# visionworkbench/visionworkbench

Hardware: AMD Instinct MI355X
Metric: disparity Mpix/s, 4096x4096 pair, 7x7 SAD, +-64-px search (higher is better)
Workload: dtype u8

## Files before the change

visionworkbench_amd/csrc/bm_sad_u8.hip:

```cpp
#include <climits>
#include <cstdlib>
#include <type_traits>

#include "vwgpu_internal.h"
#include "u8_tile.h"

#ifdef VWGPU_TILE_STAMPS
__device__ unsigned long long* g_sad_stamps = nullptr;
extern "C" int vwgpu_debug_set_sad_stamps(void* d_buf) {
  unsigned long long* p = static_cast<unsigned long long*>(d_buf);
  return hipMemcpyToSymbol(HIP_SYMBOL(g_sad_stamps), &p, sizeof p) == hipSuccess ? 0 : -3;
}
#define VWGPU_STAMP(k) do { if (g_sad_stamps && tid == 0) g_sad_stamps[(size_t)wg * 16 + (k)] = wall_clock64(); } while (0)
#else
#define VWGPU_STAMP(k) do { } while (0)
#endif

namespace {

using namespace vwgpu_u8;
typedef uint32_t u32;
typedef uint64_t u64;
typedef unsigned short u16x2 __attribute__((ext_vector_type(2)));

__device__ __forceinline__ u32 pk_sub_u16(u32 a, u32 b) {
  return __builtin_bit_cast(u32, (u16x2)(__builtin_bit_cast(u16x2, a) - __builtin_bit_cast(u16x2, b)));
}
__device__ __forceinline__ u32 pk_max_u16(u32 a, u32 b) {
  return __builtin_bit_cast(u32, __builtin_elementwise_max(__builtin_bit_cast(u16x2, a), __builtin_bit_cast(u16x2, b)));
}
__device__ __forceinline__ u32 pk_min_u16(u32 a, u32 b) {
  return __builtin_bit_cast(u32, __builtin_elementwise_min(__builtin_bit_cast(u16x2, a), __builtin_bit_cast(u16x2, b)));
}
__device__ __forceinline__ void umin3_acc(u32& k, u32 a, u32 b) {
  asm volatile("v_min3_u32 %0, %0, %1, %2" : "+v"(k) : "v"(a), "v"(b));
}

template <int W>
__device__ __forceinline__ void key_sub(u32& key, u32 a, u32 b) {
  if (W == 0)
    asm volatile("v_sub_u16_sdwa %0, %1, %2 dst_sel:WORD_1 dst_unused:UNUSED_PRESERVE src0_sel:WORD_0 src1_sel:WORD_0"
                 : "+v"(key) : "v"(a), "v"(b));
  else
    asm volatile("v_sub_u16_sdwa %0, %1, %2 dst_sel:WORD_1 dst_unused:UNUSED_PRESERVE src0_sel:WORD_1 src1_sel:WORD_1"
                 : "+v"(key) : "v"(a), "v"(b));
}

template <int KX, int KY, int TY, int WV = 0>
struct Cfg {
  static constexpr int NW = (KX + 3) / 4;
  static constexpr int EW = NW <= 2 ? 2 : 4;
  static constexpr int WAVES = WV ? WV : (NW <= 2 ? 4 : 2);
  static constexpr int THREADS = WAVES * 64;
  static constexpr int TWB = WAVES * 256;
  static constexpr int NR = TY + KY - 1;
  static constexpr int LBW = TWB / 4 + NW + 1;
  static constexpr u32 LAST_MASK = (KX % 4 == 0) ? 0xffffffffu : ((1u << (8 * (KX % 4))) - 1u);
};

__device__ __forceinline__ void divmod_small(int idx, int d, float inv, int& quo, int& rem) {
  int qq = (int)(((float)idx + 0.5f) * inv);
  int rr = idx - qq * d;
  if (rr < 0) { --qq; rr += d; }
  if (rr >= d) { ++qq; rr -= d; }
  quo = qq; rem = rr;
}

__device__ __forceinline__ bool sad_second_on_cu(unsigned block, int first_round) {
  return (int)(block >> 3) >= (first_round >> 4);
}

__host__ __device__ constexpr size_t ent_words(int nr, int ne, int ew, int gr, int ty, int pt) {
  const size_t ent = (size_t)nr * ne * ew;
  const size_t merge = gr > 1 ? (size_t)(gr - 1) * (ty / gr) * 4 * pt + (size_t)gr * pt : 0;
  const size_t ob = (size_t)gr * (pt / 64) * 768;
  return ent > merge ? (ent > ob ? ent : ob) : (merge > ob ? merge : ob);
}

template <int KX, int KY, int TY, int GR, int WV = 0, bool EM = true>
__global__ void __launch_bounds__((GR * (Cfg<KX, KY, TY, WV>::THREADS)), (GR > 1 ? 1 : (TY <= 8 && KX <= 8 ? 3 : 2)))
bm_sad_u8_kernel(const float* __restrict__ L, ptrdiff_t ls, int lw, int lh,
                 const float* __restrict__ R, ptrdiff_t rs, int rcw, int rch,
                 int sx, int sy, int ne, int32_t* __restrict__ out, ptrdiff_t os, int ow, int oh,
                 int* __restrict__ flag_set, int* __restrict__ flag_clear,
                 int gxt, int ntiles, int last_round, int first_round, int stagger_ticks) {
  typedef Cfg<KX, KY, TY, WV> C;
  constexpr bool SPLIT = GR > 1;
  constexpr int NW = C::NW, EW = C::EW, NR = C::NR;
  constexpr int NRP = EM ? (NR | 1) : NR;
  extern __shared__ __attribute__((aligned(16))) u32 lds[];
  u32* ent = lds;
  const int bpitch = ne + NW + 1;
  u32* base = lds + ent_words(NRP, ne, EW, GR, TY, C::THREADS);
  u32* item_ctr = base + (size_t)NR * bpitch;

  constexpr int PT = C::THREADS;
  constexpr int NT = GR * PT;
  const int tid = threadIdx.x;
  const int grp = SPLIT ? __builtin_amdgcn_readfirstlane(tid / PT) : 0;
  const int ltid = SPLIT ? tid % PT : tid;
  const int pair_id = __builtin_amdgcn_readfirstlane(ltid >> 6);
  const int per_xcd = gridDim.x >> 3;
  const int wg = (int)(blockIdx.x & 7) * per_xcd + (int)(blockIdx.x >> 3);
  if (wg >= ntiles) return;
  const int x0 = (wg % gxt) * C::TWB;
  const int y0 = (wg / gxt) * TY;
  const int q = x0 + 4 * ltid;
  u32 bad_acc = 0;
  if (wg == 0 && tid == 0) *flag_clear = 0;
#ifdef VWGPU_TILE_STAMPS
  if (g_sad_stamps && tid == 0) {
    unsigned hw, xcc;
    asm volatile("s_getreg_b32 %0, hwreg(HW_REG_HW_ID)" : "=s"(hw));
    asm volatile("s_getreg_b32 %0, hwreg(HW_REG_XCC_ID)" : "=s"(xcc));
    unsigned long long* rec = g_sad_stamps + (size_t)wg * 16;
    rec[0] = wall_clock64(); rec[1] = clock64(); rec[2] = ((unsigned long long)xcc << 32) | hw;
  }
#endif

  if (!SPLIT && (int)blockIdx.x < first_round && sad_second_on_cu(blockIdx.x, first_round)) {
    if (tid < 64) {
      const u64 t_start = wall_clock64();
      for (int it = 0; it < 512 && wall_clock64() - t_start < (u64)stagger_ticks; ++it) __builtin_amdgcn_s_sleep(8);
    }
    __syncthreads();
  }
  stage_u8_rows<NR>(L, ls, lw, lh, x0, y0, C::LBW, C::LBW, ent, tid, NT, bad_acc);
  stage_u8_rows<NR>(R, rs, rcw, rch, x0, y0, bpitch, bpitch, base, tid, NT, bad_acc);
  __syncthreads();
  u64 win[NR][NW];
#pragma unroll
  for (int r = 0; r < NR; ++r) {
    u32 a[NW + 1];
#pragma unroll
    for (int n = 0; n <= NW; ++n) a[n] = ent[r * C::LBW + ltid + n];
#pragma unroll
    for (int n = 0; n < NW; ++n) win[r][n] = (u64)a[n] | ((u64)a[n + 1] << 32);
  }

  VWGPU_STAMP(3);
  u32 K[TY][4];
  u32 MN[TY][2], MX[TY][2];
#pragma unroll
  for (int y = 0; y < TY; ++y) K[y][0] = K[y][1] = K[y][2] = K[y][3] = 0xffffffffu;
  u32 eq_rows = (1u << TY) - 1u;
  int eq_checks = 0;
  constexpr int NPROBE = 4;
  const u32 zero = 0;

  const bool late = !SPLIT && (int)blockIdx.x >= last_round;
  if (!SPLIT) { if (late) __builtin_amdgcn_s_setprio(2); else __builtin_amdgcn_s_setprio(3); }
  typedef std::true_type T;
  typedef std::false_type F;

  auto sweep = [&](auto max_tag) __attribute__((always_inline)) {
    constexpr bool MAXSWEEP = decltype(max_tag)::value;
    for (int dy = 0; dy < sy; ++dy) {
      __syncthreads();
      if (dy > 0 || (MAXSWEEP && sy > 1)) stage_u8_rows<NR>(R, rs, rcw, rch, x0, y0 + dy, bpitch, bpitch, base, tid, NT, bad_acc);
      for (int t = 0; t < 4; ++t) {
        const int a_last = (sx + 2 - t) >> 2;
        __syncthreads();
        if (!MAXSWEEP && !SPLIT && dy == 0 && late) {
          if (t == 2) __builtin_amdgcn_s_setprio(1);
          else if (t == 3) __builtin_amdgcn_s_setprio(0);
        }
        {
          auto build = [&](int r, int m) __attribute__((always_inline)) {
            const u32* bp = base + (size_t)r * bpitch + m;
            u32 b[NW + 1];
#pragma unroll
            for (int n = 0; n <= NW; ++n) b[n] = bp[n];
            u32 w[EW];
#pragma unroll
            for (int n = 0; n < EW; ++n) w[n] = 0;
#pragma unroll
            for (int n = 0; n < NW; ++n) w[n] = __builtin_amdgcn_alignbyte(b[n + 1], b[n], t);
            w[NW - 1] &= C::LAST_MASK;
            u32* e = ent + (EM ? (size_t)m * NRP + r : (size_t)r * ne + m) * EW;
            if (EW == 2) *reinterpret_cast<uint2*>(e) = make_uint2(w[0], w[1]);
            else *reinterpret_cast<uint4*>(e) = make_uint4(w[0], w[1], w[2 % EW], w[3 % EW]);
          };
#pragma unroll 4
          for (int r = grp; r < NR; r += NT / PT) build(r, ltid);
          const int rem = ne - PT, total = NR * rem;
          const float inv = 1.0f / (float)rem;
          for (int idx = tid; idx < total; idx += NT) {
            int r, m;
            divmod_small(idx, rem, inv, r, m);
            build(r, PT + m);
          }
          if (SPLIT && tid < PT / 64) item_ctr[tid] = 0u;
        }
        __syncthreads();

        auto step = [&](int a, auto masked_tag, auto pair_tag, auto probe_tag) __attribute__((always_inline)) {
          constexpr bool MASKED = decltype(masked_tag)::value;
          constexpr bool PAIR = decltype(pair_tag)::value;
          constexpr bool PROBE = decltype(probe_tag)::value;
          const int jbase = 4 * a + t;
          const int ibase = dy * sx + jbase;
          u32 kinA[4], kinB[4];
          u32 orA[2] = {0u, 0u};
#pragma unroll
          for (int i = 0; i < 4; ++i) {
            kinA[i] = (u32)(ibase - i) & 0xffffu;
            kinB[i] = (u32)(ibase + 4 - i) & 0xffffu;
            if (MASKED) {
              const int d = jbase - i;
              if (d < 0 || d >= sx) orA[i >> 1] |= (i & 1) ? 0xffff0000u : 0x0000ffffu;
            }
          }
          const u32* ep = ent + (size_t)(ltid + a) * (EM ? NRP * EW : EW);
          u64 accA = 0, accB = 0;
          u64 PA[NR], PB[NR];
          constexpr int PF = 4;
          u32 wa[NR][EW], wb[NR][EW];
          auto fetch = [&](int r) __attribute__((always_inline)) {
            const u32* e = ep + (EM ? (size_t)r * EW : (size_t)r * ne * EW);
            constexpr int NX = EM ? NRP * EW : EW;
            if (EW == 2) {
              const uint2 v = *reinterpret_cast<const uint2*>(e);
              wa[r][0] = v.x; wa[r][1] = v.y;
              if (PAIR) { const uint2 u = *reinterpret_cast<const uint2*>(e + NX); wb[r][0] = u.x; wb[r][1] = u.y; }
            } else {
              const uint4 v = *reinterpret_cast<const uint4*>(e);
              wa[r][0] = v.x; wa[r][1] = v.y; wa[r][2 % EW] = v.z; wa[r][3 % EW] = v.w;
              if (PAIR) { const uint4 u = *reinterpret_cast<const uint4*>(e + NX); wb[r][0] = u.x; wb[r][1] = u.y; wb[r][2 % EW] = u.z; wb[r][3 % EW] = u.w; }
            }
          };
#pragma unroll
          for (int r = 0; r < PF && r < NR; ++r) fetch(r);
#pragma unroll
          for (int r = 0; r < NR; ++r) {
            if (r + PF < NR) fetch(r + PF);
#pragma unroll
            for (int n = 0; n < NW; ++n) {
              accA = __builtin_amdgcn_qsad_pk_u16_u8(win[r][n], wa[r][n], accA);
              if (PAIR) accB = __builtin_amdgcn_qsad_pk_u16_u8(win[r][n], wb[r][n], accB);
            }
            PA[r] = accA;
            if (PAIR) PB[r] = accB;
            if (r >= KY - 1) {
              const int y = r - (KY - 1);
              const int ro = (r >= KY) ? r - KY : 0;
              const u32 nA0 = (u32)PA[r], nA1 = (u32)(PA[r] >> 32);
              const u32 oA0 = (r >= KY) ? (u32)PA[ro] : zero;
              const u32 oA1 = (r >= KY) ? (u32)(PA[ro] >> 32) : zero;
              if (MAXSWEEP) {
                const u32 sA0 = pk_sub_u16(nA0, oA0), sA1 = pk_sub_u16(nA1, oA1);
                MN[y][0] = pk_min_u16(MN[y][0], MASKED ? (sA0 | orA[0]) : sA0);
                MN[y][1] = pk_min_u16(MN[y][1], MASKED ? (sA1 | orA[1]) : sA1);
                MX[y][0] = pk_max_u16(MX[y][0], MASKED ? (sA0 & ~orA[0]) : sA0);
                MX[y][1] = pk_max_u16(MX[y][1], MASKED ? (sA1 & ~orA[1]) : sA1);
                if (PAIR) {
                  const u32 nB0 = (u32)PB[r], nB1 = (u32)(PB[r] >> 32);
                  const u32 oB0 = (r >= KY) ? (u32)PB[ro] : zero;
                  const u32 oB1 = (r >= KY) ? (u32)(PB[ro] >> 32) : zero;
                  const u32 sB0 = pk_sub_u16(nB0, oB0), sB1 = pk_sub_u16(nB1, oB1);
                  MN[y][0] = pk_min_u16(MN[y][0], sB0);
                  MN[y][1] = pk_min_u16(MN[y][1], sB1);
                  MX[y][0] = pk_max_u16(MX[y][0], sB0);
                  MX[y][1] = pk_max_u16(MX[y][1], sB1);
                }
              } else {
                key_sub<0>(kinA[0], nA0, oA0); key_sub<1>(kinA[1], nA0, oA0);
                key_sub<0>(kinA[2], nA1, oA1); key_sub<1>(kinA[3], nA1, oA1);
                if (PAIR) {
                  const u32 nB0 = (u32)PB[r], nB1 = (u32)(PB[r] >> 32);
                  const u32 oB0 = (r >= KY) ? (u32)PB[ro] : zero;
                  const u32 oB1 = (r >= KY) ? (u32)(PB[ro] >> 32) : zero;
                  key_sub<0>(kinB[0], nB0, oB0); key_sub<1>(kinB[1], nB0, oB0);
                  key_sub<0>(kinB[2], nB1, oB1); key_sub<1>(kinB[3], nB1, oB1);
                  if (PROBE) {
                    u32 x[4];
#pragma unroll
                    for (int i = 0; i < 4; ++i) {
                      asm volatile("v_xor_b32 %0, %1, %2" : "=v"(x[i]) : "v"(kinA[i]), "v"(kinB[i]));
                      x[i] = (q + i < ow) ? x[i] : 0xffffffffu;
                    }
                    const u32 m01 = x[0] < x[1] ? x[0] : x[1], m23 = x[2] < x[3] ? x[2] : x[3];
                    if ((m01 < m23 ? m01 : m23) >> 16) eq_rows &= ~(1u << y);
                  }
                  umin3_acc(K[y][0], kinA[0], kinB[0]);
                  umin3_acc(K[y][1], kinA[1], kinB[1]);
                  umin3_acc(K[y][2], kinA[2], kinB[2]);
                  umin3_acc(K[y][3], kinA[3], kinB[3]);
                } else {
                  const u32 kA0 = (MASKED && (orA[0] & 0x0000ffffu)) ? 0xffffffffu : kinA[0];
                  const u32 kA1 = (MASKED && (orA[0] & 0xffff0000u)) ? 0xffffffffu : kinA[1];
                  const u32 kA2 = (MASKED && (orA[1] & 0x0000ffffu)) ? 0xffffffffu : kinA[2];
                  const u32 kA3 = (MASKED && (orA[1] & 0xffff0000u)) ? 0xffffffffu : kinA[3];
                  umin3_acc(K[y][0], kA0, kA0);
                  umin3_acc(K[y][1], kA1, kA1);
                  umin3_acc(K[y][2], kA2, kA2);
                  umin3_acc(K[y][3], kA3, kA3);
                }
              }
            }
          }
        };

        int a_lo = (t >= 3) ? 0 : 1;
        int a_hi = (sx - 1 - t >= 0) ? ((sx - 1 - t) >> 2) + 1 : 0;
        if (a_hi > a_last + 1) a_hi = a_last + 1;
        if (a_lo > a_hi) a_lo = a_hi;
        const int n1 = a_lo;
        const int npair = (a_hi - n1) > 0 ? (a_hi - n1) >> 1 : 0;
        int nprobe = 0;
        if (!MAXSWEEP && dy == 0 && t == 0) nprobe = npair < NPROBE - eq_checks ? npair : NPROBE - eq_checks;
        const int a4 = n1 + 2 * npair;
        const int n4 = a_last - a4 + 1 > 0 ? a_last - a4 + 1 : 0;
        const int nitems = n1 + npair + n4;
        int seq = 0;
        auto next_item = [&]() __attribute__((always_inline)) -> int {
          if (MAXSWEEP) return grp == 0 ? seq++ : 0x7fffffff;
          if (!SPLIT) return seq++;
          int lane, v = 0;
          asm volatile("v_mbcnt_lo_u32_b32 %0, -1, 0\n\tv_mbcnt_hi_u32_b32 %0, -1, %0" : "=v"(lane));
          if (lane == 0) v = (int)atomicAdd(&item_ctr[pair_id], 1u);
          return __builtin_amdgcn_readfirstlane(v);
        };
        int i = next_item();
        for (; i < n1; i = next_item()) step(i, T{}, F{}, F{});
        for (; i < n1 + nprobe; i = next_item()) step(n1 + 2 * (i - n1), F{}, T{}, T{});
        for (; i < n1 + npair; i = next_item()) step(n1 + 2 * (i - n1), F{}, T{}, F{});
        for (; i < nitems; i = next_item()) step(a4 + (i - n1 - npair), T{}, F{}, F{});
        eq_checks += nprobe;
        if (!MAXSWEEP && dy == 0) VWGPU_STAMP(4 + t);
      }
    }
  };
  sweep(F{});
  if (!SPLIT) __builtin_amdgcn_s_setprio(3);

  if (bad_acc != 0u) atomicOr(flag_set, 1);
  constexpr int RG = TY / GR;
  static_assert(TY % GR == 0, "rows per group");
  auto row_mine = [&](int y) __attribute__((always_inline)) -> bool { return !SPLIT || (y / RG == grp); };
  if (SPLIT) {
    u32* xk = ent;
    u32* xe = ent + (size_t)(GR - 1) * RG * 4 * PT;
    u32 eq_all = eq_rows;
#pragma unroll
    for (int d = 0; d < GR; ++d) {
      __syncthreads();
      if (grp != d) {
        const int slot = grp < d ? grp : grp - 1;
#pragma unroll
        for (int y = 0; y < RG; ++y)
#pragma unroll
          for (int s2 = 0; s2 < 4; ++s2) xk[((slot * RG + y) * 4 + s2) * PT + ltid] = K[d * RG + y][s2];
      }
      if (d == 0) xe[grp * PT + ltid] = eq_rows;
      __syncthreads();
      if (grp == d) {
#pragma unroll
        for (int slot = 0; slot < GR - 1; ++slot)
#pragma unroll
          for (int y = 0; y < RG; ++y)
#pragma unroll
            for (int s2 = 0; s2 < 4; ++s2) {
              const u32 o = xk[((slot * RG + y) * 4 + s2) * PT + ltid];
              K[d * RG + y][s2] = o < K[d * RG + y][s2] ? o : K[d * RG + y][s2];
            }
      }
      if (d == 0) {
#pragma unroll
        for (int g2 = 0; g2 < GR; ++g2) eq_all &= xe[g2 * PT + ltid];
      }
    }
    eq_rows = eq_all;
  }
  u32 cand = eq_checks < NPROBE ? (1u << TY) - 1u : eq_rows;
#pragma unroll
  for (int y = 0; y < TY; ++y)
    if (y0 + y >= oh || q >= ow || !row_mine(y)) cand &= ~(1u << y);
  const int any = __syncthreads_or(cand != 0u);

  {
    const int wv = ltid >> 6, lane = ltid & 63;
    u32* ob = ent + (size_t)(grp * (PT / 64) + wv) * 768;
    const int xw = x0 + 256 * wv;
    int nd = (ow - xw) * 3;
    nd = nd < 0 ? 0 : (nd > 768 ? 768 : nd);
    const u32 sx_magic = sx > 1 ? (u32)(0xffffffffu / (u32)sx) + 1u : 0u;
    struct __attribute__((packed, aligned(4))) U4 { u32 x, y, z, w; };
#pragma unroll
    for (int y = 0; y < TY; ++y) {
      const int oy = y0 + y;
      if (oy >= oh || !row_mine(y)) continue;
      u32 v[12];
#pragma unroll
      for (int s = 0; s < 4; ++s) {
        const u32 di = K[y][s] & 0xffffu;
        u32 dx, dy;
        if (sy == 1) { dx = di; dy = 0; }
        else { dy = sx == 1 ? di : __umulhi(di, sx_magic); dx = di - dy * (u32)sx; }
        v[3 * s] = dx;
        v[3 * s + 1] = dy;
        v[3 * s + 2] = 0x7fffffffu;
      }
      uint4* ow4 = reinterpret_cast<uint4*>(ob + lane * 12);
      ow4[0] = make_uint4(v[0], v[1], v[2], v[3]);
      ow4[1] = make_uint4(v[4], v[5], v[6], v[7]);
      ow4[2] = make_uint4(v[8], v[9], v[10], v[11]);
      int32_t* orow = out + ((ptrdiff_t)oy * os + xw) * 3;
#pragma unroll
      for (int k = 0; k < 3; ++k) {
        const int idx = k * 256 + lane * 4;
        const uint4 t = *reinterpret_cast<const uint4*>(ob + idx);
        if (idx + 3 < nd) {
          U4 u; u.x = t.x; u.y = t.y; u.z = t.z; u.w = t.w;
          *reinterpret_cast<U4*>(orow + idx) = u;
        } else {
          if (idx < nd) orow[idx] = (int32_t)t.x;
          if (idx + 1 < nd) orow[idx + 1] = (int32_t)t.y;
          if (idx + 2 < nd) orow[idx + 2] = (int32_t)t.z;
        }
      }
    }
  }

#ifdef VWGPU_TILE_STAMPS
  if (g_sad_stamps && tid == 0) { g_sad_stamps[(size_t)wg * 16 + 8] = wall_clock64(); g_sad_stamps[(size_t)wg * 16 + 9] = clock64(); }
#endif
  if (__builtin_expect(!any, 1)) return;
#pragma unroll
  for (int y = 0; y < TY; ++y) {
    MN[y][0] = MN[y][1] = 0xffffffffu;
    MX[y][0] = MX[y][1] = 0u;
  }
  sweep(T{});
  if (grp == 0) {
#pragma unroll
    for (int y = 0; y < TY; ++y) {
      const u32 same0 = MN[y][0] ^ MX[y][0], same1 = MN[y][1] ^ MX[y][1];
      const bool inv[4] = {(same0 & 0xffffu) == 0, (same0 >> 16) == 0, (same1 & 0xffffu) == 0, (same1 >> 16) == 0};
#pragma unroll
      for (int s = 0; s < 4; ++s)
        if (inv[s] && y0 + y < oh && q + s < ow)
          out[((ptrdiff_t)(y0 + y) * os + q + s) * 3 + 2] = 0;
    }
  }
}

typedef void (*KernelFn)(const float*, ptrdiff_t, int, int, const float*, ptrdiff_t, int, int, int, int, int,
                         int32_t*, ptrdiff_t, int, int, int*, int*, int, int, int, int, int);
struct Launch {
  int kx, ky, ty;
  int threads, twb, nr, ew, nw;
  int split_groups;
  KernelFn fn;
  KernelFn split_fn;
  KernelFn fn_rm, split_fn_rm;
};

template <bool ON, int KX, int KY, int TY, int GR, int WV, bool EM>
constexpr KernelFn kernel_if() {
  if constexpr (ON) return bm_sad_u8_kernel<KX, KY, TY, GR, WV, EM>;
  else return nullptr;
}

template <int KX, int KY, int TY, bool WITH_SPLIT = false, int WV = 0>
constexpr Launch make_launch() {
  typedef Cfg<KX, KY, TY, WV> C;
  return Launch{KX, KY, TY, C::THREADS, C::TWB, C::NR, C::EW, C::NW, WV ? 4 : 2,
                kernel_if<WV == 0, KX, KY, TY, 1, WV, true>(),
                kernel_if<WITH_SPLIT, KX, KY, TY, (WV ? 4 : 2), WV, true>(),
                kernel_if<WV == 0, KX, KY, TY, 1, WV, false>(),
                kernel_if<WITH_SPLIT, KX, KY, TY, (WV ? 4 : 2), WV, false>()};
}

const Launch kLaunch[] = {
    make_launch<3, 3, 16>(), make_launch<5, 5, 16>(), make_launch<7, 7, 16, true>(), make_launch<7, 7, 8, true>(), make_launch<7, 7, 16, true, 2>(),
    make_launch<7, 5, 16>(), make_launch<9, 9, 12>(), make_launch<11, 11, 8>(),
};

const Launch* find_launch(int kx, int ky) {
  for (const Launch& l : kLaunch)
    if (l.kx == kx && l.ky == ky) return &l;
  return nullptr;
}

const Launch* pick_launch(int kx, int ky, int ow, int oh, int num_cu, int groups, bool* split) {
  const Launch* best = nullptr;
  double best_cost = 0.0;
  *split = false;
  if (groups == 3) {
    bool has = false;
    for (const Launch& l : kLaunch) has |= l.kx == kx && l.ky == ky && l.split_fn && !l.fn;
    if (!has) groups = 0;
  }
  for (const Launch& l : kLaunch) {
    if (l.kx != kx || l.ky != ky) continue;
    const long long wgs = (long long)((ow + l.twb - 1) / l.twb) * ((oh + l.ty - 1) / l.ty);
    const double n = (double)((wgs + num_cu - 1) / num_cu);
    const int resident = (l.ty <= 8 && l.kx <= 8) ? 3 : 2;
    const bool narrow = l.twb * 2 <= 4 * 256 && l.split_fn && !l.fn;
    const double wfrac = narrow ? 0.5 : 1.0;
    for (int sp = 0; sp < 2; ++sp) {
      if (sp && !l.split_fn) continue;
      if (!sp && !l.fn) continue;
      if (groups == 3 && !narrow) continue;
      if (groups && groups != 3 && (narrow || (l.split_fn && (groups == 2) != (sp == 1)))) continue;
      const double steps = (sp ? l.nr * 0.55 * n : (n < 2.0 ? l.nr * 0.74 : l.nr * 0.5 * n)) * wfrac;
      const double rounds = sp ? n : (double)(((long long)n + resident - 1) / resident);
      const double cost = steps + (narrow ? 5.7 : 4.5) * rounds;
      if (!best || cost < best_cost) { best = &l; best_cost = cost; *split = sp != 0; }
    }
  }
  return best;
}

constexpr size_t kMaxLds = 80 * 1024;

constexpr int kStaggerTicks = 1400;

int entries_per_row(const Launch& l, int sx) { return l.twb / 4 + ((sx + 2) >> 2) + 1; }

size_t lds_bytes(const Launch& l, int sx, int groups, bool em) {
  const int ne = entries_per_row(l, sx);
  const size_t ent = ent_words(em ? (l.nr | 1) : l.nr, ne, l.ew, groups, l.ty, l.threads);
  const size_t left = (size_t)l.nr * (l.twb / 4 + l.nw + 1);
  const size_t base = (size_t)l.nr * (ne + l.nw + 1);
  return ((ent > left ? ent : left) + base) * sizeof(u32);
}

bool supported(const vwgpu_bm_args& a) {
  if (a.cost_type != VWGPU_ABSOLUTE_DIFFERENCE) return false;
  const Launch* l = find_launch(a.kx, a.ky);
  if (!l) return false;
  if ((long long)a.sx * a.sy > 65535) return false;
  return lds_bytes(*l, a.sx, l->split_fn ? l->split_groups : 1, false) <= kMaxLds;
}

int launch(vwgpu_ctx* ctx, const vwgpu_bm_args& a, int** d_flag) {
  const int kx = a.kx, sx = a.sx, sy = a.sy, ow = a.ow(), oh = a.oh();
  bool split = false;
  const int plan_cu = ctx->sad_round_slots > 0 ? (ctx->sad_round_slots + 1) / 2 : ctx->num_cu;
  const Launch* l = pick_launch(kx, a.ky, ow, oh, plan_cu, ctx->sad_groups, &split);
  if (!l) return vwgpu_fail(ctx, VWGPU_ERR_NOIMPL, "no packed-u8 kernel for %dx%d", kx, a.ky);
  const int rcw = a.lw + sx - 1, rch = a.lh + sy - 1;
  const int gx = (ow + l->twb - 1) / l->twb, gy = (oh + l->ty - 1) / l->ty;
  const int ne = entries_per_row(*l, sx);
  const int groups = split ? l->split_groups : 1;
  const size_t ctr_bytes = split ? 64 : 0;
  const bool em = ctx->sad_layout == 0 && lds_bytes(*l, sx, groups, true) + ctr_bytes <= kMaxLds;
  const size_t shmem = lds_bytes(*l, sx, groups, em) + ctr_bytes;
  ctx->sad_last_launch = l->ty | (l->twb / 256) << 8 | groups << 12 | (em ? 1 : 0) << 16;
  const KernelFn main_fn = em ? (split ? l->split_fn : l->fn) : (split ? l->split_fn_rm : l->fn_rm);
  const unsigned grid1 = (unsigned)((gx * gy + 7) / 8 * 8);
  const int resident = (l->ty <= 8 && l->kx <= 8) ? 3 : 2;
  const int slots = ctx->sad_round_slots > 0 ? ctx->sad_round_slots : ctx->num_cu * resident;
  const bool rounds = !split && (int)grid1 >= 2 * slots;
  const int last_round = rounds ? (int)grid1 - slots : INT_MAX;
  const int first_round = (rounds && resident == 2) ? slots : 0;
  vwgpu_flag_pair f;
  int rc = vwgpu_packed_prologue(ctx, reinterpret_cast<const void*>(main_fn), shmem, d_flag, &f);
  if (rc) return rc;
  {
    vwgpu_prof_scope ps(ctx, "bm_sad_u8");
    hipLaunchKernelGGL(main_fn, dim3(grid1), dim3(split ? l->split_groups * l->threads : l->threads), shmem, ctx->stream,
                       a.left, a.ls, a.lw, a.lh, a.right, a.rs, rcw, rch, sx, sy, ne, a.out, a.os, ow, oh,
                       f.set, f.clear, gx, gx * gy, last_round, first_round, kStaggerTicks);
  }
  VWGPU_HIP(ctx, hipGetLastError());
  return VWGPU_OK;
}

}

vwgpu_bm_matcher vwgpu_bm_sad_u8 = {VWGPU_PATH_SAD_U8, 7, "packed-u8", supported, launch};
```

Before: 52570.

## Plan SAD disparity steps so partially masked slots pair with clean ones

For the 7x7, TY=16 configuration, the per-phase loop over disparity steps is re-planned by a new host/device helper. Edge steps that are only partly valid now use compile-time lane masks and are paired with clean steps, instead of running as separate masked single steps. This removes the runtime mask ORs and lowers the number of scheduled items per phase, including the atomic work-stealing fetches in split mode. In exchange it adds many specialised step instantiations, which grow code size and instruction-cache pressure, and probing now only happens on clean pairs.

```diff
diff --git a/visionworkbench_amd/csrc/bm_sad_u8.hip b/visionworkbench_amd/csrc/bm_sad_u8.hip
--- a/visionworkbench_amd/csrc/bm_sad_u8.hip
+++ b/visionworkbench_amd/csrc/bm_sad_u8.hip
@@ -4,6 +4,7 @@
 
 #include "vwgpu_internal.h"
 #include "u8_tile.h"
+#include "sad_items.h"
 
 #ifdef VWGPU_TILE_STAMPS
 __device__ unsigned long long* g_sad_stamps = nullptr;
@@ -86,6 +87,7 @@
                  int gxt, int ntiles, int last_round, int first_round, int stagger_ticks) {
   typedef Cfg<KX, KY, TY, WV> C;
   constexpr bool SPLIT = GR > 1;
+  constexpr bool PLAN = KX == 7 && KY == 7 && TY == 16 && GR <= 2;
   constexpr int NW = C::NW, EW = C::EW, NR = C::NR;
   constexpr int NRP = EM ? (NR | 1) : NR;
   extern __shared__ __attribute__((aligned(16))) u32 lds[];
@@ -146,6 +148,7 @@
   u32 eq_rows = (1u << TY) - 1u;
   int eq_checks = 0;
   constexpr int NPROBE = 4;
+  const int probe_budget = vwgpu_sad::probe_budget(sx, NPROBE);
   const u32 zero = 0;
 
   const bool late = !SPLIT && (int)blockIdx.x >= last_round;
@@ -194,10 +197,12 @@
         }
         __syncthreads();
 
-        auto step = [&](int a, auto masked_tag, auto pair_tag, auto probe_tag) __attribute__((always_inline)) {
+        auto step = [&](int a, auto masked_tag, auto pair_tag, auto probe_tag, auto ma_tag, auto mb_tag) __attribute__((always_inline)) {
           constexpr bool MASKED = decltype(masked_tag)::value;
           constexpr bool PAIR = decltype(pair_tag)::value;
           constexpr bool PROBE = decltype(probe_tag)::value;
+          constexpr int MA = decltype(ma_tag)::value, MB = PAIR ? decltype(mb_tag)::value : 0;
+          static_assert(!PROBE || (PAIR && !MASKED && MA == 15 && MB == 15), "only clean pairs are probed");
           const int jbase = 4 * a + t;
           const int ibase = dy * sx + jbase;
           u32 kinA[4], kinB[4];
@@ -263,55 +268,53 @@
                   MX[y][0] = pk_max_u16(MX[y][0], sB0);
                   MX[y][1] = pk_max_u16(MX[y][1], sB1);
                 }
-              } else {
+              } else if (MASKED) {
                 key_sub<0>(kinA[0], nA0, oA0); key_sub<1>(kinA[1], nA0, oA0);
                 key_sub<0>(kinA[2], nA1, oA1); key_sub<1>(kinA[3], nA1, oA1);
+                const u32 kA0 = (orA[0] & 0x0000ffffu) ? 0xffffffffu : kinA[0];
+                const u32 kA1 = (orA[0] & 0xffff0000u) ? 0xffffffffu : kinA[1];
+                const u32 kA2 = (orA[1] & 0x0000ffffu) ? 0xffffffffu : kinA[2];
+                const u32 kA3 = (orA[1] & 0xffff0000u) ? 0xffffffffu : kinA[3];
+                umin3_acc(K[y][0], kA0, kA0);
+                umin3_acc(K[y][1], kA1, kA1);
+                umin3_acc(K[y][2], kA2, kA2);
+                umin3_acc(K[y][3], kA3, kA3);
+              } else {
+                if (MA & 1) key_sub<0>(kinA[0], nA0, oA0);
+                if (MA & 2) key_sub<1>(kinA[1], nA0, oA0);
+                if (MA & 4) key_sub<0>(kinA[2], nA1, oA1);
+                if (MA & 8) key_sub<1>(kinA[3], nA1, oA1);
                 if (PAIR) {
                   const u32 nB0 = (u32)PB[r], nB1 = (u32)(PB[r] >> 32);
                   const u32 oB0 = (r >= KY) ? (u32)PB[ro] : zero;
                   const u32 oB1 = (r >= KY) ? (u32)(PB[ro] >> 32) : zero;
-                  key_sub<0>(kinB[0], nB0, oB0); key_sub<1>(kinB[1], nB0, oB0);
-                  key_sub<0>(kinB[2], nB1, oB1); key_sub<1>(kinB[3], nB1, oB1);
-                  if (PROBE) {
-                    u32 x[4];
-#pragma unroll
-                    for (int i = 0; i < 4; ++i) {
-                      asm volatile("v_xor_b32 %0, %1, %2" : "=v"(x[i]) : "v"(kinA[i]), "v"(kinB[i]));
-                      x[i] = (q + i < ow) ? x[i] : 0xffffffffu;
-                    }
-                    const u32 m01 = x[0] < x[1] ? x[0] : x[1], m23 = x[2] < x[3] ? x[2] : x[3];
-                    if ((m01 < m23 ? m01 : m23) >> 16) eq_rows &= ~(1u << y);
+                  if (MB & 1) key_sub<0>(kinB[0], nB0, oB0);
+                  if (MB & 2) key_sub<1>(kinB[1], nB0, oB0);
+                  if (MB & 4) key_sub<0>(kinB[2], nB1, oB1);
+                  if (MB & 8) key_sub<1>(kinB[3], nB1, oB1);
+                }
+                if (PROBE) {
+                  u32 x[4];
+#pragma unroll
+                  for (int i = 0; i < 4; ++i) {
+                    asm volatile("v_xor_b32 %0, %1, %2" : "=v"(x[i]) : "v"(kinA[i]), "v"(kinB[i]));
+                    x[i] = (q + i < ow) ? x[i] : 0xffffffffu;
                   }
-                  umin3_acc(K[y][0], kinA[0], kinB[0]);
-                  umin3_acc(K[y][1], kinA[1], kinB[1]);
-                  umin3_acc(K[y][2], kinA[2], kinB[2]);
-                  umin3_acc(K[y][3], kinA[3], kinB[3]);
-                } else {
-                  const u32 kA0 = (MASKED && (orA[0] & 0x0000ffffu)) ? 0xffffffffu : kinA[0];
-                  const u32 kA1 = (MASKED && (orA[0] & 0xffff0000u)) ? 0xffffffffu : kinA[1];
-                  const u32 kA2 = (MASKED && (orA[1] & 0x0000ffffu)) ? 0xffffffffu : kinA[2];
-                  const u32 kA3 = (MASKED && (orA[1] & 0xffff0000u)) ? 0xffffffffu : kinA[3];
-                  umin3_acc(K[y][0], kA0, kA0);
-                  umin3_acc(K[y][1], kA1, kA1);
-                  umin3_acc(K[y][2], kA2, kA2);
-                  umin3_acc(K[y][3], kA3, kA3);
+                  const u32 m01 = x[0] < x[1] ? x[0] : x[1], m23 = x[2] < x[3] ? x[2] : x[3];
+                  if ((m01 < m23 ? m01 : m23) >> 16) eq_rows &= ~(1u << y);
+                }
+#pragma unroll
+                for (int i = 0; i < 4; ++i) {
+                  const bool vA = (MA >> i) & 1, vB = (MB >> i) & 1;
+                  if (vA && vB) umin3_acc(K[y][i], kinA[i], kinB[i]);
+                  else if (vA) umin3_acc(K[y][i], kinA[i], kinA[i]);
+                  else if (vB) umin3_acc(K[y][i], kinB[i], kinB[i]);
                 }
               }
             }
           }
         };
 
-        int a_lo = (t >= 3) ? 0 : 1;
-        int a_hi = (sx - 1 - t >= 0) ? ((sx - 1 - t) >> 2) + 1 : 0;
-        if (a_hi > a_last + 1) a_hi = a_last + 1;
-        if (a_lo > a_hi) a_lo = a_hi;
-        const int n1 = a_lo;
-        const int npair = (a_hi - n1) > 0 ? (a_hi - n1) >> 1 : 0;
-        int nprobe = 0;
-        if (!MAXSWEEP && dy == 0 && t == 0) nprobe = npair < NPROBE - eq_checks ? npair : NPROBE - eq_checks;
-        const int a4 = n1 + 2 * npair;
-        const int n4 = a_last - a4 + 1 > 0 ? a_last - a4 + 1 : 0;
-        const int nitems = n1 + npair + n4;
         int seq = 0;
         auto next_item = [&]() __attribute__((always_inline)) -> int {
           if (MAXSWEEP) return grp == 0 ? seq++ : 0x7fffffff;
@@ -321,12 +324,73 @@
           if (lane == 0) v = (int)atomicAdd(&item_ctr[pair_id], 1u);
           return __builtin_amdgcn_readfirstlane(v);
         };
-        int i = next_item();
-        for (; i < n1; i = next_item()) step(i, T{}, F{}, F{});
-        for (; i < n1 + nprobe; i = next_item()) step(n1 + 2 * (i - n1), F{}, T{}, T{});
-        for (; i < n1 + npair; i = next_item()) step(n1 + 2 * (i - n1), F{}, T{}, F{});
-        for (; i < nitems; i = next_item()) step(a4 + (i - n1 - npair), T{}, F{}, F{});
-        eq_checks += nprobe;
+        typedef std::integral_constant<int, 15> M15;
+        if constexpr (MAXSWEEP || !PLAN) {
+          int a_lo = (t >= 3) ? 0 : 1;
+          int a_hi = (sx - 1 - t >= 0) ? ((sx - 1 - t) >> 2) + 1 : 0;
+          if (a_hi > a_last + 1) a_hi = a_last + 1;
+          if (a_lo > a_hi) a_lo = a_hi;
+          const int n1 = a_lo;
+          const int npair = (a_hi - n1) > 0 ? (a_hi - n1) >> 1 : 0;
+          int nprobe = 0;
+          if (!MAXSWEEP && dy == 0 && t == 0) nprobe = npair < NPROBE - eq_checks ? npair : NPROBE - eq_checks;
+          const int a4 = n1 + 2 * npair;
+          const int n4 = a_last - a4 + 1 > 0 ? a_last - a4 + 1 : 0;
+          const int nitems = n1 + npair + n4;
+          int i = next_item();
+          for (; i < n1; i = next_item()) step(i, T{}, F{}, F{}, M15{}, M15{});
+          if constexpr (!MAXSWEEP)
+            for (; i < n1 + nprobe; i = next_item()) step(n1 + 2 * (i - n1), F{}, T{}, T{}, M15{}, M15{});
+          for (; i < n1 + npair; i = next_item()) step(n1 + 2 * (i - n1), F{}, T{}, F{}, M15{}, M15{});
+          for (; i < nitems; i = next_item()) step(a4 + (i - n1 - npair), T{}, F{}, F{}, M15{}, M15{});
+          eq_checks += nprobe;
+        } else {
+          const vwgpu_sad::Plan pl = vwgpu_sad::plan(sx, t);
+          int i = next_item();
+          {
+            typedef std::integral_constant<int, 0> M0;
+            int nprobe = 0;
+            if (dy == 0) nprobe = pl.clean_pairs < probe_budget - eq_checks ? pl.clean_pairs : probe_budget - eq_checks;
+            const int e_hs = vwgpu_sad::end_head_single(pl), e_hp = vwgpu_sad::end_head_pair(pl), e_pr = e_hp + nprobe;
+            const int e_cp = vwgpu_sad::end_clean_pairs(pl), e_tp = vwgpu_sad::end_tail_pair(pl);
+            auto pair_a = [&](int idx) __attribute__((always_inline)) -> int { return vwgpu_sad::pair_step(pl, idx); };
+            const u32 hm = pl.head_mask;
+            typedef std::integral_constant<int, 1> M1;
+            typedef std::integral_constant<int, 3> M3;
+            typedef std::integral_constant<int, 7> M7;
+            typedef std::integral_constant<int, 8> M8;
+            typedef std::integral_constant<int, 12> M12;
+            typedef std::integral_constant<int, 14> M14;
+            for (; i < e_hs && hm == 1u; i = next_item()) step(0, F{}, F{}, F{}, M1{}, M0{});
+            for (; i < e_hs && hm == 3u; i = next_item()) step(0, F{}, F{}, F{}, M3{}, M0{});
+            for (; i < e_hs; i = next_item()) step(0, F{}, F{}, F{}, M7{}, M0{});
+            for (; i < e_hp && hm == 1u; i = next_item()) step(0, F{}, T{}, F{}, M1{}, M15{});
+            for (; i < e_hp && hm == 3u; i = next_item()) step(0, F{}, T{}, F{}, M3{}, M15{});
+            for (; i < e_hp; i = next_item()) step(0, F{}, T{}, F{}, M7{}, M15{});
+            for (; i < e_pr; i = next_item()) step(pair_a(i), F{}, T{}, T{}, M15{}, M15{});
+            for (; i < e_cp; i = next_item()) step(pair_a(i), F{}, T{}, F{}, M15{}, M15{});
+            const u32 tm = pl.tail_mask;
+            for (; i < e_tp && tm == 14u; i = next_item()) step(pair_a(i), F{}, T{}, F{}, M15{}, M14{});
+            for (; i < e_tp && tm == 12u; i = next_item()) step(pair_a(i), F{}, T{}, F{}, M15{}, M12{});
+            for (; i < e_tp; i = next_item()) step(pair_a(i), F{}, T{}, F{}, M15{}, M8{});
+            auto sa = [&](int idx) __attribute__((always_inline)) -> int { return vwgpu_sad::single_step(pl, idx); };
+            auto sm = [&](int idx) __attribute__((always_inline)) -> u32 { return pl.fallback ? vwgpu_sad::slot_mask(sx, t, idx) : tm; };
+            typedef std::integral_constant<int, 2> M2;
+            typedef std::integral_constant<int, 4> M4;
+            typedef std::integral_constant<int, 6> M6;
+            for (; i < pl.nitems && sm(i) == 1u; i = next_item()) step(sa(i), F{}, F{}, F{}, M1{}, M0{});
+            for (; i < pl.nitems && sm(i) == 3u; i = next_item()) step(sa(i), F{}, F{}, F{}, M3{}, M0{});
+            for (; i < pl.nitems && sm(i) == 7u; i = next_item()) step(sa(i), F{}, F{}, F{}, M7{}, M0{});
+            for (; i < pl.nitems && sm(i) == 2u; i = next_item()) step(sa(i), F{}, F{}, F{}, M2{}, M0{});
+            for (; i < pl.nitems && sm(i) == 4u; i = next_item()) step(sa(i), F{}, F{}, F{}, M4{}, M0{});
+            for (; i < pl.nitems && sm(i) == 6u; i = next_item()) step(sa(i), F{}, F{}, F{}, M6{}, M0{});
+            for (; i < pl.nitems && sm(i) == 15u; i = next_item()) step(sa(i), F{}, F{}, F{}, M15{}, M0{});
+            for (; i < pl.nitems && sm(i) == 14u; i = next_item()) step(sa(i), F{}, F{}, F{}, M14{}, M0{});
+            for (; i < pl.nitems && sm(i) == 12u; i = next_item()) step(sa(i), F{}, F{}, F{}, M12{}, M0{});
+            for (; i < pl.nitems && sm(i) == 8u; i = next_item()) step(sa(i), F{}, F{}, F{}, M8{}, M0{});
+            eq_checks += nprobe;
+          }
+        }
         if (!MAXSWEEP && dy == 0) VWGPU_STAMP(4 + t);
       }
     }
diff --git a/visionworkbench_amd/csrc/sad_items.h b/visionworkbench_amd/csrc/sad_items.h
--- /dev/null
+++ b/visionworkbench_amd/csrc/sad_items.h
@@ -0,0 +1,87 @@
+#pragma once
+
+#ifndef VWGPU_HD
+#define VWGPU_HD __host__ __device__
+#endif
+
+namespace vwgpu_sad {
+
+struct Item {
+  int a;
+  int pair;
+  unsigned mask_a;
+  unsigned mask_b;
+  int probe_ok;
+};
+
+struct Plan {
+  int a_last;
+  int fallback;
+  int head_single;
+  int head_pair;
+  int clean_pairs;
+  int tail_pair;
+  int tail_single;
+  unsigned head_mask, tail_mask;
+  int nitems;
+};
+
+VWGPU_HD constexpr unsigned slot_mask(int sx, int t, int a) {
+  unsigned m = 0;
+  for (int i = 0; i < 4; ++i) {
+    const int d = 4 * a + t - i;
+    if (d >= 0 && d < sx) m |= 1u << i;
+  }
+  return m;
+}
+
+VWGPU_HD constexpr int popcount4(unsigned m) { return (int)((m & 1u) + ((m >> 1) & 1u) + ((m >> 2) & 1u) + ((m >> 3) & 1u)); }
+
+VWGPU_HD constexpr Plan plan(int sx, int t) {
+  Plan p{};
+  p.a_last = (sx + 2 - t) >> 2;
+  const int nsteps = p.a_last + 1;
+  p.head_mask = slot_mask(sx, t, 0);
+  p.tail_mask = slot_mask(sx, t, p.a_last);
+  if (nsteps < 3) {
+    p.fallback = 1;
+    p.nitems = nsteps;
+    return p;
+  }
+  int first = 0, last = p.a_last;
+  if (nsteps & 1) {
+    if (popcount4(p.head_mask) < popcount4(p.tail_mask)) { p.head_single = 1; first = 1; }
+    else { p.tail_single = 1; last = p.a_last - 1; }
+  }
+  int pairs = (last - first + 1) >> 1;
+  if (!p.head_single && p.head_mask != 15u) { p.head_pair = 1; --pairs; }
+  if (!p.tail_single && p.tail_mask != 15u) { p.tail_pair = 1; --pairs; }
+  p.clean_pairs = pairs;
+  p.nitems = p.head_single + p.head_pair + p.clean_pairs + p.tail_pair + p.tail_single;
+  return p;
+}
+
+VWGPU_HD constexpr int end_head_single(const Plan& p) { return p.head_single; }
+VWGPU_HD constexpr int end_head_pair(const Plan& p) { return p.head_single + p.head_pair; }
+VWGPU_HD constexpr int end_clean_pairs(const Plan& p) { return p.head_single + p.head_pair + p.clean_pairs; }
+VWGPU_HD constexpr int end_tail_pair(const Plan& p) { return p.head_single + p.head_pair + p.clean_pairs + p.tail_pair; }
+VWGPU_HD constexpr int pair_step(const Plan& p, int idx) { return p.head_single + 2 * (idx - p.head_single); }
+
+VWGPU_HD constexpr int single_step(const Plan& p, int idx) { return p.fallback ? idx : p.a_last; }
+
+VWGPU_HD constexpr Item item(const Plan& p, int idx) {
+  if (p.fallback) return Item{idx, 0, 0u, 0u, 0};
+  if (idx < end_head_single(p)) return Item{0, 0, p.head_mask, 0u, 0};
+  if (idx < end_head_pair(p)) return Item{pair_step(p, idx), 1, p.head_mask, 15u, 0};
+  if (idx < end_clean_pairs(p)) return Item{pair_step(p, idx), 1, 15u, 15u, 1};
+  if (idx < end_tail_pair(p)) return Item{pair_step(p, idx), 1, 15u, p.tail_mask, 0};
+  return Item{p.a_last, 0, p.tail_mask, 0u, 0};
+}
+
+VWGPU_HD constexpr int probe_budget(int sx, int nprobe_max) {
+  const int a_hi = ((sx - 1) >> 2) + 1;
+  const int np = a_hi > 1 ? (a_hi - 1) >> 1 : 0;
+  return np < nprobe_max ? np : nprobe_max;
+}
+
+}
```

After: 52900, median of 6. Within noise of the previous version (+0.6%).
